# SteveMacenski/slam_toolbox

Measured on AMD Instinct MI355X. Metric: scan-matches/sec, higher is better.
Workload: dtype u8 gather / i32 sum / f64 penalty; 1 GPU; BASELINE config[1]: CorrelateScan 1081 beams 61x61x81 poses; parallelism=1 x independent match shards (no collective), streams_per_gpu=1

## Files before the change

slam_toolbox_amd/csrc/kh_internal.hpp:

```cpp
#pragma once
#include <cstddef>
#include <cstdint>

namespace kh
{

constexpr int32_t kInvalidScan = INT32_MAX;
constexpr int32_t kOccupied = 100;
constexpr int32_t kTieCap = 2048;
constexpr int32_t kGridPad = 512;
constexpr int32_t kTileBytes = 64;
constexpr int32_t kTileSpan = 61;
constexpr int32_t kClasses = 4;
constexpr int32_t kBlockShift = 5;
constexpr int32_t kCountsPerAngle = 8;
#ifndef KH_GROUP_ANGLES
#define KH_GROUP_ANGLES 2
#endif
#ifndef KH_LDS_PITCH
#define KH_LDS_PITCH 192
#endif
#ifndef KH_LDS_ROWS
#define KH_LDS_ROWS 196
#endif
#ifndef KH_LDS_REGION_KB
#define KH_LDS_REGION_KB 37
#endif
constexpr int32_t kGroupAngles = KH_GROUP_ANGLES;
constexpr int32_t kLdsRanges = 4;
inline __host__ __device__ int32_t lds_desc_capacity(int32_t n_points) {return 64 * ((n_points + 255) / 256);}
constexpr int32_t kChunkWords = 8;
static_assert(4 + kGroupAngles <= kChunkWords, "descriptor words");
constexpr int32_t kLdsPitch = KH_LDS_PITCH;
constexpr int32_t kLdsRows = KH_LDS_ROWS;
constexpr int32_t kLdsRegionBytes = KH_LDS_REGION_KB * 1024;

constexpr int32_t kMaxFootprint = 4;
constexpr uint32_t kHashEmpty = 0xffffffffu;
struct RasterJob
{
  uint8_t * grid;
  const double * const * scan_ptr;
  const int32_t * scan_prefix;
  int32_t n_scans;
  int32_t uniform_n;
  double view_x, view_y;
  uint8_t * active;
  int32_t n_points;
  int32_t ws, roi_x, roi_y, roi_w, roi_h;
  int32_t kernel_size;
  double off_x, off_y, scale;
  uint32_t * blockmap;
  int32_t bm_w, bm_h;
  int32_t bshift;
  int32_t tiles_w, tiles_h, height;
  int32_t * tile_count;
  int32_t * tile_start;
  int32_t * tile_cursor;
  int32_t * work;
  int32_t * n_work;
  int32_t * cell_xy;
  int32_t * rank;
  int32_t * list;
  int32_t n_foot;
  int32_t foot_dx[kMaxFootprint], foot_dy[kMaxFootprint];
// ... 110 lines not shown
```

slam_toolbox_amd/csrc/matcher_host.cpp:

```cpp
#include "matcher_private.hpp"
#include "matcher_seq.hpp"

namespace kh
{
thread_local std::string g_last_error;
void set_error(const std::string & s) {g_last_error = s;}
}


namespace kh
{

static int32_t half_kernel_size(double smear, double resolution)
{
  return static_cast<int32_t>(round_half_away(2.0 * smear / resolution));
}


void host_parallel_for(size_t n, const std::function<void(size_t)> & fn) {HostPool::instance().run(n, fn);}
void host_parallel_for_wide(size_t n, const std::function<void(size_t)> & fn) {HostPool::wide().run(n, fn);}
void scan_points_at(const double * ranges, size_t ranges_stride, int32_t n_beams, double min_angle, double angular_resolution, size_t n_poses,
  const double * sensor_poses, double * points, double * sensor_xy)
{
  const size_t nb = static_cast<size_t>(n_beams);
// ... 527 lines not shown
}

int ensure_slot_scratch(kh_matcher * m, const CorrReq & q, CorrHost & c, bool allow_copies)
{
  int rc = KH_OK;
  Slot & s = m->slots[c.slot];
  const size_t tp = static_cast<size_t>(c.na) * c.P;
  if (tp > s.cap_table) {
    if (s.d_table) {KH_HIP(hipStreamSynchronize(m->stream)); KH_HIP(hipFree(s.d_table)); KH_HIP(hipFree(s.d_slow));}
    const size_t cap = std::max(tp, s.cap_table + s.cap_table / 2);
    KH_HIP(hipMalloc(reinterpret_cast<void **>(&s.d_table), cap * 4));
    KH_HIP(hipMalloc(reinterpret_cast<void **>(&s.d_slow), cap * 4));
    s.cap_table = cap;
  }
  rc = ensure_device(s.d_counts, s.cap_counts, static_cast<size_t>(c.na) * kCountsPerAngle, m->stream); if (rc) {return rc;}
  {
    size_t lt = static_cast<size_t>((c.nx + 30) / 31) * ((c.ny + 4 * pick_ry(c.ny) - 1) / (4 * pick_ry(c.ny)));
    if (lt > 32) {lt = 1;}
    c.lt_alloc = static_cast<int32_t>(lt);
    rc = ensure_device(s.d_fast, s.cap_fast, 2 * tp * kClasses * lt, m->stream); if (rc) {return rc;}
    rc = ensure_device(s.d_tcounts, s.cap_tcounts, 2 * static_cast<size_t>(c.na) * kClasses * lt, m->stream); if (rc) {return rc;}
    const double work = static_cast<double>(c.nx) * c.ny * c.na * c.P;
    const double cells_per_step = q.res_x * m->scale;
    const bool full_res = c.nx > 1 && std::fabs(cells_per_step - 1.0) < 1e-9 && c.nx <= kTileSpan;
    const bool tiled_lists = lt > 1 && (std::fabs(cells_per_step - 1.0) < 1e-9 || std::fabs(cells_per_step - 2.0) < 1e-9);
    if (allow_copies && m->dual_copy && !s.d_grid2 && (full_res || tiled_lists) && work >= 1e8) {
      const bool two_cells = std::fabs(cells_per_step - 2.0) < 1e-9 && m->copy_q > 0 && (m->ws % 8) == 0;
      rc = allocate_copies(m, s, two_cells ? 2 : 1); if (rc) {return rc;}
    }
  }
  {
    const size_t groups = (static_cast<size_t>(c.na) + kGroupAngles - 1) / kGroupAngles;
    const size_t range_len = static_cast<size_t>(lds_desc_capacity(c.P));
    rc = ensure_device(s.d_chunks, s.cap_chunks, groups * kLdsRanges * range_len * kChunkWords, m->stream); if (rc) {return rc;}
    rc = ensure_device(s.d_chunk_counts, s.cap_chunk_counts, groups * kLdsRanges, m->stream); if (rc) {return rc;}
  }
  const size_t vol = static_cast<size_t>(c.nx) * c.ny * c.na;
  rc = ensure_device(s.d_sums, s.cap_volume, vol, m->stream); if (rc) {return rc;}
  rc = ensure_device(s.d_tile_best, s.cap_tile_best,
      static_cast<size_t>(c.na) * ((c.nx + 30) / 31) * ((c.ny + 3) / 4), m->stream); if (rc) {return rc;}
  if (m->keep_responses) {rc = ensure_device(s.d_resp, s.cap_resp, vol, m->stream); if (rc) {return rc;}}

  return KH_OK;
}

void prepare_job(kh_matcher * m, const CorrReq & q, CorrHost & c, const StageLayout & L, uint8_t * hb, uint8_t * db,
  unsigned long long * d_out, size_t out_words, size_t n_launch, bool lds_always, bool lds_never, JobShape & shape)
{
  const kh_match_params & mp = m->params;
  Slot & s = m->slots[c.slot];
  CorrJob * job = reinterpret_cast<CorrJob *>(hb);
  int32_t * bx = reinterpret_cast<int32_t *>(hb + L.bx);
  int32_t * by = reinterpret_cast<int32_t *>(hb + L.by);
  double * ang_pen = reinterpret_cast<double *>(hb + L.ang_pen);
  double * cos_sin = reinterpret_cast<double *>(hb + L.cos_sin);
  double * local = reinterpret_cast<double *>(hb + L.local);
  uint8_t * invalid = hb + L.invalid;

  c.bx.resize(c.nx); c.by.resize(c.ny);
  for (int32_t k = 0; k < c.nx; ++k) {
    const double newPositionX = c.center[0] + c.geo->x_poses[k];
    const double gx = (newPositionX - s.off_x) * m->scale;
    c.bx[k] = to_int32(round_half_away(gx)) + m->roi_x;
    bx[k] = c.bx[k];
  }
  for (int32_t k = 0; k < c.ny; ++k) {
    const double newPositionY = c.center[1] + c.geo->y_poses[k];
    const double gy = (newPositionY - s.off_y) * m->scale;
// ... 323 lines not shown
      const CorrJob * job = reinterpret_cast<const CorrJob *>(B.h_stage + stride * i);
      launch_score(B.d_stage + stride * i, stride, 1, job->tiles_x * job->tiles_y, job->na,
        (job->linear && job->sx == 2 && !job->dec) ? 2 : 1, job->ry, cs);
    }
  }
  if (m->profiling) {KH_HIP(hipEventRecord(B.ev[1], cs)); KH_HIP(hipEventRecord(B.evs[2], cs));}
  launch_ties(B.d_stage, stride, static_cast<int32_t>(n), max_poses, tile_pairs, B.use_lds, cs);
  if (m->profiling) {KH_HIP(hipEventRecord(B.evs[3], cs));}
  KH_HIP(hipGetLastError());
  KH_HIP(hipMemcpyAsync(B.h_out, B.d_out, out_words * 8 * n, hipMemcpyDeviceToHost, cs));
  size_t max_small = 0;
  for (size_t i = 0; i < n; ++i) {
    const size_t vol = static_cast<size_t>(B.ctx[i].nx) * B.ctx[i].ny * B.ctx[i].na;
    if (B.ctx[i].fine && vol <= kSmallVolume) {max_small = std::max(max_small, vol);}
  }
  B.small_stride = align_up(max_small, 32);
  if (max_small) {
    rc = ensure_pinned(B.h_sums, B.cap_hsums, B.small_stride * n, m->stream); if (rc) {return rc;}
    rc = ensure_device(B.d_small, B.cap_dsmall, B.small_stride * n, m->stream); if (rc) {return rc;}
    launch_gather_small(B.d_stage, stride, static_cast<int32_t>(n), B.d_small, static_cast<int32_t>(B.small_stride), cs);
    KH_HIP(hipMemcpyAsync(B.h_sums, B.d_small, B.small_stride * n * 4, hipMemcpyDeviceToHost, cs));
  }
  KH_HIP(hipEventRecord(B.done, cs));
  timing.lap(1, t_enqueue);
  return KH_OK;
}

static int dump_lds_chunks(const kh_matcher * m, const CorrBatch & B)
{
  const CorrHost & c0 = B.ctx[0];
  const Slot & s0 = m->slots[c0.slot];
  const size_t groups = (static_cast<size_t>(c0.na) + kGroupAngles - 1) / kGroupAngles;
  const size_t range_len = static_cast<size_t>(lds_desc_capacity(c0.P));
  std::vector<int32_t> cc(groups * kLdsRanges), dd(groups * kLdsRanges * range_len * kChunkWords);
  KH_HIP(hipMemcpy(cc.data(), s0.d_chunk_counts, cc.size() * 4, hipMemcpyDeviceToHost));
  KH_HIP(hipMemcpy(dd.data(), s0.d_chunks, dd.size() * 4, hipMemcpyDeviceToHost));
  long total = 0, bytes = 0, windows = 0, maxb = 0, small = 0;
  for (size_t g = 0; g < groups * kLdsRanges; ++g) {
    for (int32_t k = 0; k < cc[g]; ++k) {
      const int32_t * d = dd.data() + (g * range_len + k) * kChunkWords;
      ++total; bytes += static_cast<long>(d[2]) * kLdsPitch; windows += d[3];
      maxb = std::max<long>(maxb, static_cast<long>(d[2]) * kLdsPitch);
      if (d[3] < 16) {++small;}
    }
  }
  std::fprintf(stderr, "[kh lds] job 0: %zu angle pairs, %ld chunks (%.1f per pair, %ld with < 16 windows), mean region %.1f KB, max %.1f KB, "
    "%.1f windows per chunk, %.0f staged bytes per window\n",
    groups, total, static_cast<double>(total) / groups, small, bytes / 1024.0 / std::max(1l, total), maxb / 1024.0,
    static_cast<double>(windows) / std::max(1l, total), static_cast<double>(bytes) / std::max(1l, windows));
  return KH_OK;
}

static int finish_chunk(kh_matcher * m, CorrReq * reqs, size_t n, CorrBatch & B, bool last_of_call)
{
  if (n == 0) {return KH_OK;}
  StageTiming & timing = stage_timing();
  const auto t_enter = std::chrono::steady_clock::now();
  constexpr uint64_t kAwaitResults = 200 * HostPool::kTicksPerMicrosecond, kAwaitNextCall = 120 * HostPool::kTicksPerMicrosecond;
  if (last_of_call) {HostPool::instance().run(2, [](size_t) {}, kAwaitResults);}
  KH_HIP(hipEventSynchronize(B.done));
  timing.lap(2, t_enter);
  const auto t_final = std::chrono::steady_clock::now();
  if (B.use_lds && std::getenv("KH_LDS_DEBUG")) {
    const int rc = dump_lds_chunks(m, B); if (rc) {return rc;}
  }
  if (m->profiling) {
    float ms = 0;
    KH_HIP(hipEventElapsedTime(&ms, B.ev[0], B.ev[1]));
    m->score_ms += ms; m->score_launches += 1; m->score_jobs += static_cast<int64_t>(n);
    KH_HIP(hipEventElapsedTime(&ms, B.evs[0], B.evs[1])); m->offsets_ms += ms;
    KH_HIP(hipEventElapsedTime(&ms, B.evs[2], B.evs[3])); m->ties_ms += ms;
  }

  std::vector<int> final_rc(n, KH_OK);
  auto finalize = [&](size_t i) -> int {
    const CorrHost & c = B.ctx[i];
    ResultView v;
    v.out = B.h_out + B.out_words * i;
    const size_t vol = static_cast<size_t>(c.nx) * c.ny * c.na;
    v.small = (c.fine && vol <= kSmallVolume && B.h_sums) ? B.h_sums + B.small_stride * i : nullptr;
    v.h_job = reinterpret_cast<CorrJob *>(B.h_stage + B.stride * i); v.d_job = B.d_stage + B.stride * i; v.stride = B.stride;
    return finalize_job(m, reqs[i], B.ctx[i], v);
// ... 707 lines not shown
```

slam_toolbox_amd/csrc/matcher_kernels.hip:

```cpp
#include <hip/hip_runtime.h>
#include <algorithm>
#include <atomic>
#include <cstdint>
#include <cstdlib>
#include "kh_internal.hpp"
#include "matcher_device.hpp"

namespace kh
{

constexpr int kCodeWords = 128;
__global__ __launch_bounds__(64) void k_find_valid_lane(const RasterJob * jobs, const ValidItem * items, int n_items)
{
  __shared__ uint32_t s_codes[kCodeWords][64];
  const int t = blockIdx.x * blockDim.x + threadIdx.x;
  if (t >= n_items) {return;}
  const int lane = threadIdx.x;
  const RasterJob & job = jobs[items[t].job];
  const int k = items[t].scan;
  const int n = job.scan_prefix[k + 1] - job.scan_prefix[k];
  const double2 * pts = reinterpret_cast<const double2 *>(job.scan_ptr[k]);
  uint8_t * out = job.active + job.scan_prefix[k];
  const bool in_lds = n <= 16 * kCodeWords;
  const double vx = job.view_x, vy = job.view_y;
  const double min_square_distance = 0.1 * 0.1;
  double fx = 0.0, fy = 0.0;
  bool first_time = true;
  constexpr int kAhead = 8;
  uint32_t word = 0;
  for (int base = 0; base < n; base += kAhead) {
    double2 c[kAhead];
#pragma unroll
    for (int u = 0; u < kAhead; ++u) {c[u] = pts[min(base + u, n - 1)];}
#pragma unroll
    for (int u = 0; u < kAhead; ++u) {
      const int it = base + u;
      if (it >= n) {break;}
      const double cx = c[u].x, cy = c[u].y;
// ... 1253 lines not shown
          const double delta = response - best;
          const bool tie = delta < 0.0 ? delta >= -1e-06 : delta <= 1e-06;
          if (tie) {
            const unsigned long long slot = atomicAdd(&job.out[1], 1ull);
            if (slot < (unsigned long long)kTieCap) {tie_idx[slot] = (uint32_t)((size_t)p * na + a);}
          }
        }
      }
    }
    __syncthreads();
  }
}

void launch_ties(const uint8_t * d_jobs, size_t stride, int32_t n_jobs, int32_t max_poses, int32_t tile_pairs, bool cells_in_score, void * stream)
{
  if (n_jobs <= 0 || max_poses <= 0) {return;}
  if (cells_in_score) {
    hipLaunchKernelGGL(k_ties_only, dim3(n_jobs >= 16 ? 4 : 16, n_jobs), dim3(256), 0, (hipStream_t)stream, d_jobs, stride);
    return;
  }
  int blocks = (max_poses + 255) / 256;
  if (tile_pairs > 0) {blocks = std::min(tile_pairs, n_jobs >= 16 ? 16 : 64);}
  if (blocks > 1024) {blocks = 1024;}
  hipLaunchKernelGGL(k_ties, dim3(blocks, n_jobs), dim3(256), 0, (hipStream_t)stream, d_jobs, stride);
}

}

namespace kh
{

struct ChunkDesc {int32_t beam_begin, g0, rows, windows, cnt[kChunkWords - 4];};
static_assert(sizeof(ChunkDesc) == kChunkWords * 4, "descriptor size");
static_assert(kGroupAngles >= 2 && kGroupAngles <= 4, "K3' runs kGroupAngles x 4 waves: at most 1024 threads");
static_assert(kLdsPitch % 16 == 0 && kLdsPitch % 128 == 64, "rows of a 32-lane half must fall into disjoint banks");
static_assert(kLdsRegionBytes % 1024 == 0 && kLdsRegionBytes >= kLdsRows * kLdsPitch, "one LDS-DMA instruction fills 1 KB");

constexpr int kNotFast = INT32_MIN;

template <bool kMin>
__device__ __forceinline__ int wave_prefix(int v)
{
  constexpr int ident = kMin ? INT32_MAX : INT32_MIN;
  auto op = [](int x, int y) {return kMin ? (y < x ? y : x) : (y > x ? y : x);};
  v = op(v, __builtin_amdgcn_update_dpp(ident, v, 0x111, 0xf, 0xf, false));
  v = op(v, __builtin_amdgcn_update_dpp(ident, v, 0x112, 0xf, 0xf, false));
  v = op(v, __builtin_amdgcn_update_dpp(ident, v, 0x114, 0xf, 0xf, false));
  v = op(v, __builtin_amdgcn_update_dpp(ident, v, 0x118, 0xf, 0xf, false));
  v = op(v, __builtin_amdgcn_update_dpp(ident, v, 0x142, 0xa, 0xf, false));
  v = op(v, __builtin_amdgcn_update_dpp(ident, v, 0x143, 0xc, 0xf, false));
  return v;
}
__device__ __forceinline__ int wave_prefix_min(int v, int) {return wave_prefix<true>(v);}
__device__ __forceinline__ int wave_prefix_max(int v, int) {return wave_prefix<false>(v);}

__global__ __launch_bounds__(256) void k_offsets_lds(const uint8_t * jobs, size_t stride)
{
  const CorrJob & job = *reinterpret_cast<const CorrJob *>(jobs + (size_t)blockIdx.y * stride);
  const int group = blockIdx.x;
  const int a0 = group * kGroupAngles;
  if (a0 >= job.na) {return;}
  {
    const int groups = (job.na + kGroupAngles - 1) / kGroupAngles;
    const int per = (job.out_words + groups - 1) / groups;
    const int hi = min(job.out_words, (group + 1) * per);
    for (int i = group * per + threadIdx.x; i < hi; i += blockDim.x) {job.out[i] = 0ull;}
  }
  const int P = job.n_points;
  __shared__ int32_t s_slow[kGroupAngles];
  if (threadIdx.x < kGroupAngles) {s_slow[threadIdx.x] = 0;}
  const uint32_t * const bmp = job.blockmap;
  __syncthreads();
  const int lane = threadIdx.x & 63, wave = threadIdx.x >> 6;
  const int64_t bmin = job.base0;
  const int64_t bmax = (int64_t)job.base0 + (int64_t)(job.nx - 1) * job.sx + (int64_t)(job.ny - 1) * job.sy_ws;
  const int32_t xs = (job.nx - 1) * job.sx + 1, ys = (job.ny - 1) * job.sy_cells + 1;
  const int ws = job.ws, bm_w = job.bm_w, bm_h = job.bm_h, bshift = job.bshift, na = job.na, base0 = job.base0;
  const float inv_ws = 1.0f / (float)ws;
  const int64_t data_size = job.data_size, pad = job.pad;
  const double off_x = job.grid_off_x, off_y = job.grid_off_y, scale = job.scale;
  const int row_waves = lds_row_waves(job.ny);
  const int read_rows = (16 * row_waves - 1) * job.sy_cells + 1;
  const int span_rows = ys;
  double cosine[kGroupAngles], sine[kGroupAngles];
#pragma unroll
  for (int q = 0; q < kGroupAngles; ++q) {
    cosine[q] = a0 + q < na ? job.cos_sin[2 * (a0 + q)] : 1.0;
    sine[q] = a0 + q < na ? job.cos_sin[2 * (a0 + q) + 1] : 0.0;
  }
  int32_t * const table = job.table;
  int32_t * const slow = job.slow;
  int32_t * const rel_out = job.rel;
  const int rounds = (P + 255) / 256;
  const int desc_cap = lds_desc_capacity(P);
  ChunkDesc * out = reinterpret_cast<ChunkDesc *>(job.chunks) + ((size_t)group * kLdsRanges + wave) * desc_cap;
  int n_out = 0;
  long long windows_total = 0;
  constexpr int kMaxRounds = 8;
  double plx[kMaxRounds], ply[kMaxRounds];
  bool pinv[kMaxRounds];
  {
    typedef __attribute__((address_space(1))) const uint8_t gflag;
    typedef __attribute__((address_space(1))) const double gdouble;
    gflag * const ginvalid = (gflag *)job.invalid;
    gdouble * const glocal = (gdouble *)job.local;
    uint8_t fl[kMaxRounds];
#pragma unroll
    for (int t = 0; t < kMaxRounds; ++t) {
      const int ic = min((int)threadIdx.x + 256 * t, P - 1);
      fl[t] = ginvalid[ic]; plx[t] = glocal[2 * ic]; ply[t] = glocal[2 * ic + 1];
    }
#pragma unroll
    for (int t = 0; t < kMaxRounds; ++t) {
      const int i = threadIdx.x + 256 * t;
      const bool in = t < rounds && i < P;
      pinv[t] = in ? fl[t] != 0 : true;
      plx[t] = in ? plx[t] : 0.0;
      ply[t] = in ? ply[t] : 0.0;
    }
  }
#pragma unroll
  for (int t = 0; t < kMaxRounds; ++t) {
    if (t >= rounds) {break;}
    const int i = threadIdx.x + 256 * t;
    const bool inr = i < P;
    int gx[kGroupAngles], gy[kGroupAngles];
#pragma unroll
    for (int q = 0; q < kGroupAngles; ++q) {
// ... 57 lines not shown
        const int al = (int)(((int64_t)base0 + xmin) & 15);
        const int px0 = xmin - al;
        const bool fits = any && (xmax - px0 + kTileBytes <= kLdsPitch) && (ymax - ymin + read_rows <= kLdsRows);
        const unsigned long long okm = __ballot(!any || fits) | ((1ull << begin) - 1ull);
        const int first_bad = (okm == ~0ull) ? 64 : __ffsll((long long)~okm) - 1;
        n = first_bad - begin;
        if (n > 0) {
          x0 = __shfl(px0, first_bad - 1); y0 = __shfl(ymin, first_bad - 1);
          rows = __shfl(ymax, first_bad - 1) - y0 + span_rows;
          any_chunk = __shfl((int)any, first_bad - 1) != 0;
          break;
        }
        if (lane == begin) {
          int qd = 0;
#pragma unroll
          for (int q = 1; q < kGroupAngles; ++q) {qd = gy[q] != kNotFast ? q : qd;}
#pragma unroll
          for (int q = 0; q < kGroupAngles; ++q) {
            if (q == qd) {
              (slow + (size_t)(a0 + q) * P)[atomicAdd(&s_slow[q], 1)] = gx[q] + gy[q] * ws;
              gy[q] = kNotFast;
            }
          }
        }
      }
      n = min(n, n_run - begin);
      if (any_chunk) {
        const bool in = lane >= begin && lane < begin + n;
        ChunkDesc d;
        d.beam_begin = run_lo + begin;
        d.g0 = y0 * ws + x0; d.rows = rows;
#pragma unroll
        for (int q = kGroupAngles; q < kChunkWords - 4; ++q) {d.cnt[q] = 0;}
        int windows = 0;
#pragma unroll
        for (int q = 0; q < kGroupAngles; ++q) {
          const int a = a0 + q;
          d.cnt[q] = 0;
          if (a >= na) {continue;}
          const bool mine = in && gy[q] != kNotFast;
          const int rel = (gy[q] - y0) * kLdsPitch + (gx[q] - x0);
          const int cls = rel & 3;
          int offset = 0, my_rank = 0, packed = 0;
#pragma unroll
          for (int c = 0; c < kClasses; ++c) {
            const unsigned long long mask = __ballot(mine && cls == c);
            const int cnt = __popcll(mask);
            if (cls == c) {my_rank = offset + __popcll(mask & ((1ull << lane) - 1ull));}
            offset += cnt;
            packed |= cnt << (8 * c);
          }
          d.cnt[q] = packed;
          windows += offset;
          if (mine) {rel_out[(size_t)a * P + run_lo + begin + my_rank] = rel & ~3;}
        }
        d.windows = windows;
        windows_total += windows;
        if (lane == 0) {out[n_out] = d;}
        ++n_out;
      }
      begin += n;
    }
  }
  if (lane == 0) {
    job.chunk_counts[(size_t)group * kLdsRanges + wave] = n_out;
    if (job.load_counter && windows_total) {atomicAdd(job.load_counter, (unsigned long long)(windows_total * 4 * row_waves));}
  }
  __syncthreads();
  if (threadIdx.x < kGroupAngles && a0 + (int)threadIdx.x < job.na) {
    job.counts[kCountsPerAngle * (a0 + threadIdx.x) + kClasses] = s_slow[threadIdx.x];
  }
}

void launch_offsets_lds(const uint8_t * d_jobs, size_t stride, int32_t n_jobs, int32_t max_na, void * stream)
{
  if (n_jobs <= 0 || max_na <= 0) {return;}
  const int groups = (max_na + kGroupAngles - 1) / kGroupAngles;
  hipLaunchKernelGGL(k_offsets_lds, dim3(groups, n_jobs), dim3(256), 0, (hipStream_t)stream, d_jobs, stride);
}

typedef __attribute__((address_space(3))) uint32_t lds_u32;
typedef __attribute__((address_space(1))) const void gvoid;
typedef int v4i __attribute__((ext_vector_type(4)));

#ifndef KH_PRIO
#define KH_PRIO 1
#endif
constexpr int kScoreLdsBlocksPerCu = (160 * 1024 - 4096) / (2 * kLdsRegionBytes);
constexpr int kTilePoses = 64 * kTileSpan;
static_assert(kGroupAngles * kTilePoses * 4 + (kGroupAngles - 1) * kTilePoses * 8 <= 2 * kLdsRegionBytes,
  "the sums and the exchanged responses of kGroupAngles angles must fit the workgroup's two LDS regions");
static_assert((kGroupAngles * kTilePoses * 4) % 8 == 0, "the exchanged responses are doubles");
static_assert(kScoreLdsBlocksPerCu >= 1 && kScoreLdsBlocksPerCu * kGroupAngles * 4 <= 16, "four waves per SIMD");
template <int S, int NW, bool kFull>
__global__ __launch_bounds__(64 * kGroupAngles * NW, 4) void k_score_lds(const uint8_t * jobs, size_t stride, int n_jobs, int groups_max, int xcd_map)
{
  constexpr int RQ = 16 / NW;
  constexpr int kThreadsPerAngle = 64 * NW;
  constexpr int PX = (S == 1) ? kTileSpan : (kTileSpan + 1) / 2;
  constexpr int kRowStep = 4 * S * kLdsPitch;
  int job_index, group;
  if (xcd_map) {
    const int xcd = blockIdx.x & 7, qb = blockIdx.x >> 3;
    job_index = (qb / groups_max) * 8 + xcd;
// ... 7 lines not shown
  if (group * kGroupAngles >= job.na) {return;}
  extern __shared__ __attribute__((aligned(16))) uint32_t s_region[];
  const int tid = threadIdx.x;
  const int lane = tid & 63;
  const int wave = __builtin_amdgcn_readfirstlane(tid >> 6);
  const int lx = lane & 15, ly = lane >> 4;
  const int q = wave / NW, quarter = wave % NW;
  const int row_waves = kFull ? NW : lds_row_waves(job.ny) * (NW / 4);
  const int parts = kFull ? 1 : NW / row_waves;
  const int share = kFull ? quarter : quarter % row_waves, part = kFull ? 0 : quarter / row_waves;
  const int a = group * kGroupAngles + q;
  const bool live = a < job.na;
  const int P = job.n_points;
  const int range_len = lds_desc_capacity(P);

  v4i acc[kClasses][RQ];
#pragma unroll
  for (int c = 0; c < kClasses; ++c) {
#pragma unroll
    for (int r = 0; r < RQ; ++r) {acc[c][r] = v4i{0, 0, 0, 0};}
  }
  v4i sel;
  {
    const int i = lane & 15;
    const int one = ((lane >> 4) == (i >> 2)) ? (int)(0x01010101u & (0xffu << (8 * (i & 3)))) : 0;
    sel = v4i{one, one, one, one};
  }
  const int lanebase = 4 * lx + (4 * RQ * share + ly) * S * kLdsPitch;

  const gbyte * gwin = as_global(job.grid) + job.base0;
  const gint * grel = as_global(job.rel + (size_t)(live ? a : 0) * P);
  typedef const __attribute__((address_space(4))) int32_t cint;
  cint * cdescs = (cint *)(job.chunks + (size_t)group * kLdsRanges * range_len * kChunkWords);
  cint * ccounts = (cint *)(job.chunk_counts + (size_t)group * kLdsRanges);
  struct Chunk {int beam_begin, g0, rows, packed;};

  constexpr int kUnitsPerRow = kLdsPitch / 16;
  constexpr int kWaves = kGroupAngles * NW;
  constexpr int kDmaPerWave = (kLdsRegionBytes / 1024 + kWaves - 1) / kWaves;
  const int ws = job.ws;
  uint32_t dma_off[kDmaPerWave];
#pragma unroll
  for (int t = 0; t < kDmaPerWave; ++t) {
    const int u = 64 * (wave + kWaves * t) + lane;
    const int row = u / kUnitsPerRow, col = u - row * kUnitsPerRow;
    dma_off[t] = (uint32_t)(row * ws + 16 * col);
  }
  auto issue_dma = [&](const Chunk & d, int buf) {
    const gbyte * src = gwin + d.g0;
    const int nblk = (d.rows * kUnitsPerRow + 63) >> 6;
    const uint32_t o_last = (uint32_t)((d.rows - 1) * ws + 16 * (kUnitsPerRow - 1));
    lds_u32 * dst = (lds_u32 *)s_region + buf * (kLdsRegionBytes / 4) + wave * 256;
#pragma unroll
    for (int t = 0; t < kDmaPerWave; ++t) {
      if (wave + kWaves * t >= nblk) {break;}
      const uint32_t o = dma_off[t] < o_last ? dma_off[t] : o_last;
      __builtin_amdgcn_global_load_lds((gvoid *)(src + o), (__attribute__((address_space(3))) void *)(dst + kWaves * t * 256), 16, 0, 0);
    }
  };
  auto load_rel = [&](const Chunk & d) -> int32_t {
    const int cnt = (d.packed & 0xff) + ((d.packed >> 8) & 0xff) + ((d.packed >> 16) & 0xff) + ((d.packed >> 24) & 0xff);
    return (live && lane < cnt) ? grel[d.beam_begin + lane] : 0;
  };
  const uint32_t lds_base = (uint32_t)(uintptr_t)(__attribute__((address_space(3))) char *)((char *)s_region);
  const uint32_t lds_lane = lds_base + (uint32_t)lanebase;
#define KH_DSR(dst, addr, r) asm volatile("ds_read_b32 %0, %1 offset:%2" : "=v"(dst) : "v"(addr), "n"((r) * kRowStep) : "memory")
#define KH_STEP(selector) do { \
    int32_t w[RQ][4]; \
    _Pragma("unroll") for (int r = 0; r < RQ; ++r) {KH_DSR(w[r][0], a0, r); KH_DSR(w[r][1], a1, r); KH_DSR(w[r][2], a2, r); KH_DSR(w[r][3], a3, r);} \
    if (RQ == 4) { \
      asm volatile("s_waitcnt lgkmcnt(0)" : "+v"(w[0][0]), "+v"(w[0][1]), "+v"(w[0][2]), "+v"(w[0][3]), "+v"(w[1][0]), "+v"(w[1][1]), "+v"(w[1][2]), "+v"(w[1][3]), \
        "+v"(w[RQ - 2][0]), "+v"(w[RQ - 2][1]), "+v"(w[RQ - 2][2]), "+v"(w[RQ - 2][3]), "+v"(w[RQ - 1][0]), "+v"(w[RQ - 1][1]), "+v"(w[RQ - 1][2]), "+v"(w[RQ - 1][3])); \
    } else { \
      asm volatile("s_waitcnt lgkmcnt(0)" : "+v"(w[0][0]), "+v"(w[0][1]), "+v"(w[0][2]), "+v"(w[0][3]), "+v"(w[1][0]), "+v"(w[1][1]), "+v"(w[1][2]), "+v"(w[1][3])); \
    } \
    _Pragma("unroll") for (int r = 0; r < RQ; ++r) { \
      acc[c][r] = __builtin_amdgcn_mfma_i32_16x16x64_i8(selector, (v4i{w[r][0], w[r][1], w[r][2], w[r][3]}), acc[c][r], 0, 0, 0); \
    } \
  } while (0)
  int step_base = 0;
  auto score = [&](const Chunk & d, int buf, int32_t rels) {
    if (!live) {return;}
    const uint32_t base = lds_lane + (uint32_t)(buf * kLdsRegionBytes);
    int off = 0;
#pragma unroll
    for (int c = 0; c < kClasses; ++c) {
      const int cnt = (d.packed >> (8 * c)) & 0xff;
      const int first = kFull ? 0 : (part - step_base) & (parts - 1);
      if (!kFull) {step_base += (cnt + 3) >> 2;}
      int k = 4 * first;
      for (; k + 4 <= cnt; k += 4 * parts) {
        const int i0 = off + k;
        const uint32_t a0 = base + (uint32_t)__builtin_amdgcn_readlane(rels, i0);
        const uint32_t a1 = base + (uint32_t)__builtin_amdgcn_readlane(rels, i0 + 1);
        const uint32_t a2 = base + (uint32_t)__builtin_amdgcn_readlane(rels, i0 + 2);
        const uint32_t a3 = base + (uint32_t)__builtin_amdgcn_readlane(rels, i0 + 3);
        KH_STEP(sel);
      }
      if (k < cnt) {
        const int i0 = off + k, rem = cnt - k;
        const uint32_t a0 = base + (uint32_t)__builtin_amdgcn_readlane(rels, i0);
        const uint32_t a1 = base + (uint32_t)__builtin_amdgcn_readlane(rels, rem > 1 ? i0 + 1 : i0);
        const uint32_t a2 = base + (uint32_t)__builtin_amdgcn_readlane(rels, rem > 2 ? i0 + 2 : i0);
        const uint32_t a3 = a0;
        const v4i sel_tail = v4i{sel[0], rem > 1 ? sel[1] : 0, rem > 2 ? sel[2] : 0, 0};
        KH_STEP(sel_tail);
      }
      off += cnt;
    }
  };
#undef KH_STEP
#undef KH_DSR

  static_assert(kLdsRanges == 4, "the four chunk counts are held in scalar registers");
  const int end0 = ccounts[0], end1 = end0 + ccounts[1], end2 = end1 + ccounts[2], n_chunks = end2 + ccounts[3];
  int fetched = 0;
  auto next_chunk = [&](Chunk & d) -> bool {
    if (fetched >= n_chunks) {return false;}
    const int range = (fetched >= end0 ? 1 : 0) + (fetched >= end1 ? 1 : 0) + (fetched >= end2 ? 1 : 0);
    const int start = fetched >= end2 ? end2 : fetched >= end1 ? end1 : fetched >= end0 ? end0 : 0;
    cint * w = cdescs + ((size_t)range * range_len + (fetched - start)) * kChunkWords;
    d.beam_begin = w[0]; d.g0 = w[1]; d.rows = w[2]; d.packed = w[4 + q];
    ++fetched;
    return true;
  };
  Chunk cur = {0, 0, 0, 0}, nxt = {0, 0, 0, 0}, aft = {0, 0, 0, 0};
  bool have = next_chunk(cur);
  bool more = have && next_chunk(nxt);
  int buf = 0;
  int32_t rel_cur = 0, rel_nxt = 0;
  if (have) {issue_dma(cur, 0); rel_cur = load_rel(cur);}
  while (have) {
    __syncthreads();
    if (more) {issue_dma(nxt, buf ^ 1); rel_nxt = load_rel(nxt);}
    const bool after = more && next_chunk(aft);
    __builtin_amdgcn_s_setprio(KH_PRIO);
    score(cur, buf, rel_cur);
    __builtin_amdgcn_s_setprio(0);
    cur = nxt; nxt = aft; rel_cur = rel_nxt; buf ^= 1; have = more; more = after;
  }
  __syncthreads();

  const size_t plane = (size_t)job.nx * job.ny;
  const int ta = tid % kThreadsPerAngle;
  int32_t * s_tile = reinterpret_cast<int32_t *>(s_region) + q * (64 * PX);
  if (S == 1 && kFull) {
    if (live) {
#pragma unroll
      for (int r = 0; r < RQ; ++r) {
        int32_t * const row = s_tile + (4 * RQ * share + 4 * r + ly) * PX + 4 * lx;
#pragma unroll
        for (int b = 0; b < 4; ++b) {
          int32_t total = acc[0][r][b];
#pragma unroll
          for (int c = 1; c < kClasses; ++c) {
            const int32_t v = acc[c][r][(b + c) & 3];
            total += (b + c) < 4 ? v : __builtin_amdgcn_update_dpp(0, v, 0x101, 0xf, 0xf, true);
          }
          if (4 * lx + b < PX) {row[b] = total;}
        }
      }
    }
  } else {
    for (int i = ta; i < 64 * PX; i += kThreadsPerAngle) {s_tile[i] = 0;}
    __syncthreads();
    if (live) {
#pragma unroll
      for (int c = 0; c < kClasses; ++c) {
#pragma unroll
        for (int r = 0; r < RQ; ++r) {
#pragma unroll
          for (int b = 0; b < 4; ++b) {
            const int j = 4 * lx + b;
            const int x = (j - c) / S;
            const bool pose = j >= c && ((j - c) % S) == 0 && x < PX;
            if (pose && acc[c][r][b] != 0) {atomicAdd(&s_tile[(4 * RQ * share + 4 * r + ly) * PX + x], acc[c][r][b]);}
          }
        }
      }
    }
  }
  constexpr int kPosesPerThread = (64 * PX + kThreadsPerAngle - 1) / kThreadsPerAngle;
  const int nx = job.nx, ny = job.ny;
  const bool penal = job.do_penalize != 0, wr_resp = job.write_resp != 0;
  const double denom = job.denom;
  int32_t * const sums_out = job.sums + (size_t)(live ? a : 0) * plane;
  double * const resp_out = wr_resp ? job.resp + (size_t)(live ? a : 0) * plane : nullptr;
  const int32_t * const jbx = job.bx, * const jby = job.by;
  const uint8_t * const jgrid = job.grid;
  const int64_t data_size = job.data_size;
  constexpr int kOwned = (kPosesPerThread + kGroupAngles - 1) / kGroupAngles;
  constexpr int kRounds = kOwned * kGroupAngles;
  const bool cells = job.coarse != 0 && job.cells_in_score != 0;
  typedef __attribute__((address_space(1))) unsigned long long gu64;
  gu64 * const probs = (gu64 *)(job.out + kOutHeaderWords);
  double * const s_xch = reinterpret_cast<double *>(reinterpret_cast<int32_t *>(s_region) + kGroupAngles * kTilePoses);
  auto slab_of = [&](int owner) -> int {return kGroupAngles == 2 ? 0 : (q - owner + kGroupAngles) % kGroupAngles - 1;};
  double dpen[kRounds];
  const double apen = (live && penal) ? job.ang_pen[a] : 1.0;
#pragma unroll
  for (int k = 0; k < kRounds; ++k) {
    const int p = ta + kThreadsPerAngle * k;
    const int yi = p / PX, xi = p % PX;
    dpen[k] = (live && penal && xi < nx && yi < ny) ? job.dist_pen[yi * nx + xi] : 1.0;
  }
  double mine[kOwned];
#pragma unroll
  for (int j = 0; j < kOwned; ++j) {mine[j] = 0.0;}
  __syncthreads();
  const int n_slow = live ? job.counts[kCountsPerAngle * a + kClasses] : 0;
  const int32_t * slow = job.slow + (size_t)(live ? a : 0) * P;
  double best = 0.0;
#pragma unroll
  for (int k = 0; k < kRounds; ++k) {
    const int p = ta + kThreadsPerAngle * k;
    const int yi = p / PX, xi = p % PX;
    if (xi >= nx || yi >= ny) {continue;}
    const bool owned = k % kGroupAngles == q;
    double response = 0.0;
    if (live) {
      int32_t sum = s_tile[p];
      if (n_slow > 0) {
        const int64_t pose = (int64_t)jbx[xi] + (int64_t)jby[yi];
        for (int j = 0; j < n_slow; ++j) {
          const int64_t idx = pose + slow[j];
          if (idx >= 0 && idx < data_size) {sum += jgrid[idx];}
        }
      }
      const size_t o = (size_t)yi * nx + xi;
      sums_out[o] = sum;
      response = (double)sum / denom;
      if (penal) {
        const double delta = response - 0.0;
        const bool is_zero = delta < 0.0 ? delta >= -1e-06 : delta <= 1e-06;
        if (!is_zero) {response *= (dpen[k] * apen);}
      }
      if (wr_resp) {resp_out[o] = response;}
      best = response > best ? response : best;
    }
    if (cells) {
      if (owned) {mine[k / kGroupAngles] = response;} else {s_xch[slab_of(k % kGroupAngles) * kTilePoses + p] = response;}
    }
  }
  unsigned long long seen[kOwned];
  uint32_t cell[kOwned];
  constexpr uint32_t kNoCell = 0xffffffffu;
#pragma unroll
  for (int j = 0; j < kOwned; ++j) {
    const int p = ta + kThreadsPerAngle * (kGroupAngles * j + q);
    const int yi = p / PX, xi = p % PX;
    cell[j] = (cells && xi < nx && yi < ny) ? (uint32_t)(yi * nx + xi) : kNoCell;
    __builtin_assume(cell[j] == kNoCell || cell[j] < 64u * kTileSpan);
    seen[j] = cell[j] != kNoCell ? __hip_atomic_load(probs + cell[j], __ATOMIC_RELAXED, __HIP_MEMORY_SCOPE_AGENT) : 0ull;
  }
#pragma unroll
  for (int sft = 32; sft > 0; sft >>= 1) {
    const double o = __shfl_xor(best, sft);
    best = o > best ? o : best;
  }
  __shared__ double s_best[kGroupAngles * NW];
  if (lane == 0) {s_best[wave] = best;}
  __syncthreads();
  if (live && ta == 0) {
    const double * wb = s_best + NW * q;
    double b = wb[0];
#pragma unroll
    for (int t = 1; t < NW; ++t) {b = wb[t] > b ? wb[t] : b;}
    if (job.tile_best) {job.tile_best[a] = b;}
    if (b > 0.0) {atomicMax(&job.out[0], (unsigned long long)__double_as_longlong(b));}
  }
  if (cells) {
    bool raise[kOwned];
#pragma unroll
    for (int j = 0; j < kOwned; ++j) {
      const int p = ta + kThreadsPerAngle * (kGroupAngles * j + q);
      raise[j] = false;
      if (cell[j] == kNoCell) {continue;}
#pragma unroll
      for (int t = 0; t < kGroupAngles - 1; ++t) {
        const double o = s_xch[t * kTilePoses + p];
        mine[j] = o > mine[j] ? o : mine[j];
      }
      raise[j] = (unsigned long long)__double_as_longlong(mine[j]) > seen[j];
    }
#pragma unroll
    for (int j = 0; j < kOwned; ++j) {
      if (raise[j]) {
        (void)__hip_atomic_fetch_max(probs + cell[j], (unsigned long long)__double_as_longlong(mine[j]), __ATOMIC_RELAXED, __HIP_MEMORY_SCOPE_AGENT);
      }
    }
  }
}

void launch_score_lds(const uint8_t * d_jobs, size_t stride, int32_t n_jobs, int32_t max_na, int32_t sx_variant, bool full_rows, void * stream)
{
  if (n_jobs <= 0 || max_na <= 0) {return;}
  const int groups = (max_na + kGroupAngles - 1) / kGroupAngles;
  const int xcd_map = n_jobs >= 8 ? 1 : 0;
  const int jobs_per_xcd = (n_jobs + 7) / 8;
  const long long blocks = xcd_map ? 8ll * jobs_per_xcd * groups : (long long)n_jobs * groups;
  constexpr int kDyn = 2 * kLdsRegionBytes;
  static std::atomic<unsigned long long> attr_done[4] = {{0}, {0}, {0}, {0}};
// ... 16 lines not shown
```

Baseline: 120,400 scan-matches/s.

## Stage LDS chunks through a variable-size ring with deeper DMA prefetch

Replaces the fixed double-buffered LDS staging in the scoring kernel with a ring allocator that places each chunk by its actual size. This lets up to two chunks be prefetched ahead using counted vmcnt waits instead of full syncthreads. The offsets kernel now compacts the per-wave descriptor lists into one flat list per group, and precomputes DMA unit counts and last offsets so each descriptor arrives in one scalar load. Relative-offset loads also move to LDS via DMA, and the cell atomic loads are hoisted earlier. This adds a compaction pass, doubles the descriptor buffer, and relies on hand-tuned wait counts and ring-overlap logic, which could race if the accounting is wrong.

```diff
diff --git a/slam_toolbox_amd/csrc/kh_internal.hpp b/slam_toolbox_amd/csrc/kh_internal.hpp
--- a/slam_toolbox_amd/csrc/kh_internal.hpp
+++ b/slam_toolbox_amd/csrc/kh_internal.hpp
@@ -29,8 +29,8 @@
 constexpr int32_t kGroupAngles = KH_GROUP_ANGLES;
 constexpr int32_t kLdsRanges = 4;
 inline __host__ __device__ int32_t lds_desc_capacity(int32_t n_points) {return 64 * ((n_points + 255) / 256);}
-constexpr int32_t kChunkWords = 8;
-static_assert(4 + kGroupAngles <= kChunkWords, "descriptor words");
+constexpr int32_t kChunkWords = kGroupAngles <= 2 ? 8 : 16;
+static_assert(4 + kGroupAngles + 2 <= kChunkWords, "descriptor words");
 constexpr int32_t kLdsPitch = KH_LDS_PITCH;
 constexpr int32_t kLdsRows = KH_LDS_ROWS;
 constexpr int32_t kLdsRegionBytes = KH_LDS_REGION_KB * 1024;
diff --git a/slam_toolbox_amd/csrc/lds_ring.hpp b/slam_toolbox_amd/csrc/lds_ring.hpp
--- /dev/null
+++ b/slam_toolbox_amd/csrc/lds_ring.hpp
@@ -0,0 +1,27 @@
+#pragma once
+#include <cstdint>
+
+#if defined(__HIPCC__)
+#define KH_RING_FN __host__ __device__ inline
+#else
+#define KH_RING_FN inline
+#endif
+
+namespace kh
+{
+
+struct RingPlace {int32_t unit; bool fits;};
+
+KH_RING_FN RingPlace lds_ring_place(int32_t ring_half, int32_t off_old, int32_t n_old, int32_t off_new, int32_t n_new, int32_t n)
+{
+  int32_t at = n_new > 0 ? off_new + n_new : 0;
+  if (at < ring_half && at + n > ring_half) {at = ring_half;}
+  if (at + n > 2 * ring_half) {at = 0;}
+  const bool hits_old = n_old > 0 && at < off_old + n_old && off_old < at + n;
+  const bool hits_new = n_new > 0 && at < off_new + n_new && off_new < at + n;
+  return RingPlace{at, !hits_old && !hits_new};
+}
+
+KH_RING_FN int32_t lds_ring_units(int32_t rows, int32_t pitch) {return (rows * pitch + 1023) >> 10;}
+
+}
diff --git a/slam_toolbox_amd/csrc/matcher_host.cpp b/slam_toolbox_amd/csrc/matcher_host.cpp
--- a/slam_toolbox_amd/csrc/matcher_host.cpp
+++ b/slam_toolbox_amd/csrc/matcher_host.cpp
@@ -583,8 +583,8 @@
   {
     const size_t groups = (static_cast<size_t>(c.na) + kGroupAngles - 1) / kGroupAngles;
     const size_t range_len = static_cast<size_t>(lds_desc_capacity(c.P));
-    rc = ensure_device(s.d_chunks, s.cap_chunks, groups * kLdsRanges * range_len * kChunkWords, m->stream); if (rc) {return rc;}
-    rc = ensure_device(s.d_chunk_counts, s.cap_chunk_counts, groups * kLdsRanges, m->stream); if (rc) {return rc;}
+    rc = ensure_device(s.d_chunks, s.cap_chunks, 2 * groups * kLdsRanges * range_len * kChunkWords, m->stream); if (rc) {return rc;}
+    rc = ensure_device(s.d_chunk_counts, s.cap_chunk_counts, groups, m->stream); if (rc) {return rc;}
   }
   const size_t vol = static_cast<size_t>(c.nx) * c.ny * c.na;
   rc = ensure_device(s.d_sums, s.cap_volume, vol, m->stream); if (rc) {return rc;}
@@ -974,13 +974,14 @@
   const Slot & s0 = m->slots[c0.slot];
   const size_t groups = (static_cast<size_t>(c0.na) + kGroupAngles - 1) / kGroupAngles;
   const size_t range_len = static_cast<size_t>(lds_desc_capacity(c0.P));
-  std::vector<int32_t> cc(groups * kLdsRanges), dd(groups * kLdsRanges * range_len * kChunkWords);
+  const size_t group_len = kLdsRanges * range_len;
+  std::vector<int32_t> cc(groups), dd(groups * group_len * kChunkWords);
   KH_HIP(hipMemcpy(cc.data(), s0.d_chunk_counts, cc.size() * 4, hipMemcpyDeviceToHost));
   KH_HIP(hipMemcpy(dd.data(), s0.d_chunks, dd.size() * 4, hipMemcpyDeviceToHost));
   long total = 0, bytes = 0, windows = 0, maxb = 0, small = 0;
-  for (size_t g = 0; g < groups * kLdsRanges; ++g) {
+  for (size_t g = 0; g < groups; ++g) {
     for (int32_t k = 0; k < cc[g]; ++k) {
-      const int32_t * d = dd.data() + (g * range_len + k) * kChunkWords;
+      const int32_t * d = dd.data() + (g * group_len + k) * kChunkWords;
       ++total; bytes += static_cast<long>(d[2]) * kLdsPitch; windows += d[3];
       maxb = std::max<long>(maxb, static_cast<long>(d[2]) * kLdsPitch);
       if (d[3] < 16) {++small;}
@@ -990,6 +991,14 @@
     "%.1f windows per chunk, %.0f staged bytes per window\n",
     groups, total, static_cast<double>(total) / groups, small, bytes / 1024.0 / std::max(1l, total), maxb / 1024.0,
     static_cast<double>(windows) / std::max(1l, total), static_cast<double>(bytes) / std::max(1l, windows));
+  for (size_t g = 0; g < groups; ++g) {
+    std::fprintf(stderr, "[kh lds] job 0 pair %zu:", g);
+    for (int32_t k = 0; k < cc[g]; ++k) {
+      const int32_t * d = dd.data() + (g * group_len + k) * kChunkWords;
+      std::fprintf(stderr, " %d:%d:%d:%d:%d", d[0], d[2], d[3], d[kChunkWords - 2], d[kChunkWords - 1]);
+    }
+    std::fprintf(stderr, "\n");
+  }
   return KH_OK;
 }
 
diff --git a/slam_toolbox_amd/csrc/matcher_kernels.hip b/slam_toolbox_amd/csrc/matcher_kernels.hip
--- a/slam_toolbox_amd/csrc/matcher_kernels.hip
+++ b/slam_toolbox_amd/csrc/matcher_kernels.hip
@@ -4,6 +4,7 @@
 #include <cstdint>
 #include <cstdlib>
 #include "kh_internal.hpp"
+#include "lds_ring.hpp"
 #include "matcher_device.hpp"
 
 namespace kh
@@ -1323,6 +1324,7 @@
 
 struct ChunkDesc {int32_t beam_begin, g0, rows, windows, cnt[kChunkWords - 4];};
 static_assert(sizeof(ChunkDesc) == kChunkWords * 4, "descriptor size");
+constexpr int kDescUnits = kChunkWords - 2, kDescLast = kChunkWords - 1;
 static_assert(kGroupAngles >= 2 && kGroupAngles <= 4, "K3' runs kGroupAngles x 4 waves: at most 1024 threads");
 static_assert(kLdsPitch % 16 == 0 && kLdsPitch % 128 == 64, "rows of a 32-lane half must fall into disjoint banks");
 static_assert(kLdsRegionBytes % 1024 == 0 && kLdsRegionBytes >= kLdsRows * kLdsPitch, "one LDS-DMA instruction fills 1 KB");
@@ -1359,6 +1361,7 @@
   }
   const int P = job.n_points;
   __shared__ int32_t s_slow[kGroupAngles];
+  __shared__ int32_t s_nout[kLdsRanges];
   if (threadIdx.x < kGroupAngles) {s_slow[threadIdx.x] = 0;}
   const uint32_t * const bmp = job.blockmap;
   __syncthreads();
@@ -1384,7 +1387,9 @@
   int32_t * const rel_out = job.rel;
   const int rounds = (P + 255) / 256;
   const int desc_cap = lds_desc_capacity(P);
-  ChunkDesc * out = reinterpret_cast<ChunkDesc *>(job.chunks) + ((size_t)group * kLdsRanges + wave) * desc_cap;
+  const int groups_all = (na + kGroupAngles - 1) / kGroupAngles;
+  ChunkDesc * const flat = reinterpret_cast<ChunkDesc *>(job.chunks) + (size_t)group * kLdsRanges * desc_cap;
+  ChunkDesc * out = reinterpret_cast<ChunkDesc *>(job.chunks) + ((size_t)(groups_all + group) * kLdsRanges + wave) * desc_cap;
   int n_out = 0;
   long long windows_total = 0;
   constexpr int kMaxRounds = 8;
@@ -1508,6 +1513,8 @@
         d.g0 = y0 * ws + x0; d.rows = rows;
 #pragma unroll
         for (int q = kGroupAngles; q < kChunkWords - 4; ++q) {d.cnt[q] = 0;}
+        d.cnt[kDescUnits - 4] = lds_ring_units(rows, kLdsPitch);
+        d.cnt[kDescLast - 4] = (rows - 1) * ws + 16 * (kLdsPitch / 16 - 1);
         int windows = 0;
 #pragma unroll
         for (int q = 0; q < kGroupAngles; ++q) {
@@ -1539,13 +1546,28 @@
     }
   }
   if (lane == 0) {
-    job.chunk_counts[(size_t)group * kLdsRanges + wave] = n_out;
+    s_nout[wave] = n_out;
     if (job.load_counter && windows_total) {atomicAdd(job.load_counter, (unsigned long long)(windows_total * 4 * row_waves));}
   }
   __syncthreads();
   if (threadIdx.x < kGroupAngles && a0 + (int)threadIdx.x < job.na) {
     job.counts[kCountsPerAngle * (a0 + threadIdx.x) + kClasses] = s_slow[threadIdx.x];
   }
+  int before = 0, total = 0;
+#pragma unroll
+  for (int w = 0; w < kLdsRanges; ++w) {
+    const int n = s_nout[w];
+    before += w < wave ? n : 0; total += n;
+  }
+  {
+    typedef int v4i32 __attribute__((ext_vector_type(4)));
+    static_assert(sizeof(ChunkDesc) % 16 == 0, "descriptors are moved 16 bytes at a time");
+    constexpr int kPer = sizeof(ChunkDesc) / 16;
+    const v4i32 * const src = reinterpret_cast<const v4i32 *>(out);
+    v4i32 * const dst = reinterpret_cast<v4i32 *>(flat + before);
+    for (int k = lane; k < kPer * n_out; k += 64) {dst[k] = src[k];}
+  }
+  if (threadIdx.x == 0) {job.chunk_counts[group] = total;}
 }
 
 void launch_offsets_lds(const uint8_t * d_jobs, size_t stride, int32_t n_jobs, int32_t max_na, void * stream)
@@ -1619,8 +1641,9 @@
   const gint * grel = as_global(job.rel + (size_t)(live ? a : 0) * P);
   typedef const __attribute__((address_space(4))) int32_t cint;
   cint * cdescs = (cint *)(job.chunks + (size_t)group * kLdsRanges * range_len * kChunkWords);
-  cint * ccounts = (cint *)(job.chunk_counts + (size_t)group * kLdsRanges);
-  struct Chunk {int beam_begin, g0, rows, packed;};
+  const int n_chunks = ((cint *)job.chunk_counts)[group];
+  const int n_slow = live ? ((cint *)job.counts)[kCountsPerAngle * a + kClasses] : 0;
+  struct Chunk {int beam_begin, g0, cnt[kGroupAngles], units, o_last, at;};
 
   constexpr int kUnitsPerRow = kLdsPitch / 16;
   constexpr int kWaves = kGroupAngles * NW;
@@ -1633,22 +1656,24 @@
     const int row = u / kUnitsPerRow, col = u - row * kUnitsPerRow;
     dma_off[t] = (uint32_t)(row * ws + 16 * col);
   }
-  auto issue_dma = [&](const Chunk & d, int buf) {
+  __shared__ int32_t s_rel[3][kGroupAngles][64];
+  const int rel_last = P - 1;
+  auto issue_dma = [&](const Chunk & d, int slot) {
+    if (live && quarter == 0) {
+      const int i = min(d.beam_begin + lane, rel_last);
+      __builtin_amdgcn_global_load_lds((gvoid *)(grel + i), (__attribute__((address_space(3))) void *)&s_rel[slot][q][0], 4, 0, 0);
+    }
     const gbyte * src = gwin + d.g0;
-    const int nblk = (d.rows * kUnitsPerRow + 63) >> 6;
-    const uint32_t o_last = (uint32_t)((d.rows - 1) * ws + 16 * (kUnitsPerRow - 1));
-    lds_u32 * dst = (lds_u32 *)s_region + buf * (kLdsRegionBytes / 4) + wave * 256;
+    const uint32_t o_last = (uint32_t)d.o_last;
+    lds_u32 * dst = (lds_u32 *)s_region + d.at * 256 + wave * 256;
 #pragma unroll
     for (int t = 0; t < kDmaPerWave; ++t) {
-      if (wave + kWaves * t >= nblk) {break;}
+      if (wave + kWaves * t >= d.units) {break;}
       const uint32_t o = dma_off[t] < o_last ? dma_off[t] : o_last;
       __builtin_amdgcn_global_load_lds((gvoid *)(src + o), (__attribute__((address_space(3))) void *)(dst + kWaves * t * 256), 16, 0, 0);
     }
   };
-  auto load_rel = [&](const Chunk & d) -> int32_t {
-    const int cnt = (d.packed & 0xff) + ((d.packed >> 8) & 0xff) + ((d.packed >> 16) & 0xff) + ((d.packed >> 24) & 0xff);
-    return (live && lane < cnt) ? grel[d.beam_begin + lane] : 0;
-  };
+  auto dma_pieces = [&](const Chunk & d) -> int {return max(0, (d.units - wave + kWaves - 1) / kWaves);};
   const uint32_t lds_base = (uint32_t)(uintptr_t)(__attribute__((address_space(3))) char *)((char *)s_region);
   const uint32_t lds_lane = lds_base + (uint32_t)lanebase;
 #define KH_DSR(dst, addr, r) asm volatile("ds_read_b32 %0, %1 offset:%2" : "=v"(dst) : "v"(addr), "n"((r) * kRowStep) : "memory")
@@ -1666,13 +1691,16 @@
     } \
   } while (0)
   int step_base = 0;
-  auto score = [&](const Chunk & d, int buf, int32_t rels) {
+  auto score = [&](const Chunk & d, int32_t rels) {
     if (!live) {return;}
-    const uint32_t base = lds_lane + (uint32_t)(buf * kLdsRegionBytes);
+    int packed = d.cnt[0];
+#pragma unroll
+    for (int t = 1; t < kGroupAngles; ++t) {packed = q == t ? d.cnt[t] : packed;}
+    const uint32_t base = lds_lane + (uint32_t)(d.at * 1024);
     int off = 0;
 #pragma unroll
     for (int c = 0; c < kClasses; ++c) {
-      const int cnt = (d.packed >> (8 * c)) & 0xff;
+      const int cnt = (packed >> (8 * c)) & 0xff;
       const int first = kFull ? 0 : (part - step_base) & (parts - 1);
       if (!kFull) {step_base += (cnt + 3) >> 2;}
       int k = 4 * first;
@@ -1699,37 +1727,82 @@
 #undef KH_STEP
 #undef KH_DSR
 
-  static_assert(kLdsRanges == 4, "the four chunk counts are held in scalar registers");
-  const int end0 = ccounts[0], end1 = end0 + ccounts[1], end2 = end1 + ccounts[2], n_chunks = end2 + ccounts[3];
+  constexpr int kRingHalf = kLdsRegionBytes / 1024;
+  static_assert(kDmaPerWave <= 5, "the counted waits below");
+  typedef int v8i __attribute__((ext_vector_type(8)));
+  static_assert(kChunkWords == 8, "a descriptor is one scalar load of eight words");
   int fetched = 0;
   auto next_chunk = [&](Chunk & d) -> bool {
     if (fetched >= n_chunks) {return false;}
-    const int range = (fetched >= end0 ? 1 : 0) + (fetched >= end1 ? 1 : 0) + (fetched >= end2 ? 1 : 0);
-    const int start = fetched >= end2 ? end2 : fetched >= end1 ? end1 : fetched >= end0 ? end0 : 0;
-    cint * w = cdescs + ((size_t)range * range_len + (fetched - start)) * kChunkWords;
-    d.beam_begin = w[0]; d.g0 = w[1]; d.rows = w[2]; d.packed = w[4 + q];
+    const v8i w = *(const __attribute__((address_space(4))) v8i *)(cdescs + (size_t)fetched * kChunkWords);
+    d.beam_begin = w[0]; d.g0 = w[1];
+#pragma unroll
+    for (int t = 0; t < kGroupAngles; ++t) {d.cnt[t] = w[4 + t];}
+    d.units = w[kDescUnits]; d.o_last = w[kDescLast]; d.at = 0;
     ++fetched;
     return true;
   };
-  Chunk cur = {0, 0, 0, 0}, nxt = {0, 0, 0, 0}, aft = {0, 0, 0, 0};
-  bool have = next_chunk(cur);
-  bool more = have && next_chunk(nxt);
-  int buf = 0;
-  int32_t rel_cur = 0, rel_nxt = 0;
-  if (have) {issue_dma(cur, 0); rel_cur = load_rel(cur);}
-  while (have) {
-    __syncthreads();
-    if (more) {issue_dma(nxt, buf ^ 1); rel_nxt = load_rel(nxt);}
-    const bool after = more && next_chunk(aft);
+  const uint32_t rel_lane = (uint32_t)(uintptr_t)(__attribute__((address_space(3))) char *)((char *)&s_rel[0][q][lane]);
+  Chunk c0 = {}, c1 = c0, c2 = c0, c3 = c0;
+  bool h0 = next_chunk(c0);
+  bool h1 = h0 && next_chunk(c1);
+  bool h2 = h1 && next_chunk(c2);
+  bool issued1 = false;
+  int slot = 0;
+  int ahead = 0;
+  if (h0) {issue_dma(c0, 0);}
+  while (h0) {
+    switch (ahead) {
+      case 0: asm volatile("s_waitcnt vmcnt(0)" ::: "memory"); break;
+      case 1: asm volatile("s_waitcnt vmcnt(1)" ::: "memory"); break;
+      case 2: asm volatile("s_waitcnt vmcnt(2)" ::: "memory"); break;
+      case 3: asm volatile("s_waitcnt vmcnt(3)" ::: "memory"); break;
+      case 4: asm volatile("s_waitcnt vmcnt(4)" ::: "memory"); break;
+      default: asm volatile("s_waitcnt vmcnt(5)" ::: "memory"); break;
+    }
+    __builtin_amdgcn_s_barrier();
+    int32_t rels;
+    asm volatile("ds_read_b32 %0, %1" : "=v"(rels) : "v"(rel_lane + (uint32_t)(slot * (int)sizeof(s_rel[0]))) : "memory");
+    const bool h3 = h2 && next_chunk(c3);
+    const int slot1 = slot == 2 ? 0 : slot + 1, slot2 = slot1 == 2 ? 0 : slot1 + 1;
+    if (h1 && !issued1) {
+      c1.at = lds_ring_place(kRingHalf, 0, 0, c0.at, c0.units, c1.units).unit;
+      issue_dma(c1, slot1);
+    }
+    ahead = 0;
+    bool issued2 = false;
+    if (h2) {
+      const RingPlace place = lds_ring_place(kRingHalf, c0.at, c0.units, c1.at, c1.units, c2.units);
+      if (place.fits) {c2.at = place.unit; issue_dma(c2, slot2); ahead = dma_pieces(c2); issued2 = true;}
+    }
+    asm volatile("s_waitcnt lgkmcnt(0)" : "+v"(rels) :: "memory");
     __builtin_amdgcn_s_setprio(KH_PRIO);
-    score(cur, buf, rel_cur);
+    score(c0, rels);
     __builtin_amdgcn_s_setprio(0);
-    cur = nxt; nxt = aft; rel_cur = rel_nxt; buf ^= 1; have = more; more = after;
+    c0 = c1; c1 = c2; c2 = c3; h0 = h1; h1 = h2; h2 = h3; issued1 = issued2; slot = slot1;
   }
   __syncthreads();
 
-  const size_t plane = (size_t)job.nx * job.ny;
+  const __attribute__((address_space(4))) CorrJob & cj = *(const __attribute__((address_space(4))) CorrJob *)(jobs + (size_t)job_index * stride);
+  const int nx = cj.nx, ny = cj.ny;
+  const size_t plane = (size_t)nx * ny;
   const int ta = tid % kThreadsPerAngle;
+  constexpr int kPosesPerThread = (64 * PX + kThreadsPerAngle - 1) / kThreadsPerAngle;
+  constexpr int kOwned = (kPosesPerThread + kGroupAngles - 1) / kGroupAngles;
+  const bool cells = cj.coarse != 0 && cj.cells_in_score != 0;
+  typedef __attribute__((address_space(1))) unsigned long long gu64;
+  gu64 * const probs = (gu64 *)(cj.out + kOutHeaderWords);
+  unsigned long long seen[kOwned];
+  uint32_t cell[kOwned];
+  constexpr uint32_t kNoCell = 0xffffffffu;
+#pragma unroll
+  for (int j = 0; j < kOwned; ++j) {
+    const int p = ta + kThreadsPerAngle * (kGroupAngles * j + q);
+    const int yi = p / PX, xi = p % PX;
+    cell[j] = (cells && xi < nx && yi < ny) ? (uint32_t)(yi * nx + xi) : kNoCell;
+    __builtin_assume(cell[j] == kNoCell || cell[j] < 64u * kTileSpan);
+    seen[j] = cell[j] != kNoCell ? __hip_atomic_load(probs + cell[j], __ATOMIC_RELAXED, __HIP_MEMORY_SCOPE_AGENT) : 0ull;
+  }
   int32_t * s_tile = reinterpret_cast<int32_t *>(s_region) + q * (64 * PX);
   if (S == 1 && kFull) {
     if (live) {
@@ -1767,36 +1840,38 @@
       }
     }
   }
-  constexpr int kPosesPerThread = (64 * PX + kThreadsPerAngle - 1) / kThreadsPerAngle;
-  const int nx = job.nx, ny = job.ny;
-  const bool penal = job.do_penalize != 0, wr_resp = job.write_resp != 0;
-  const double denom = job.denom;
-  int32_t * const sums_out = job.sums + (size_t)(live ? a : 0) * plane;
-  double * const resp_out = wr_resp ? job.resp + (size_t)(live ? a : 0) * plane : nullptr;
-  const int32_t * const jbx = job.bx, * const jby = job.by;
-  const uint8_t * const jgrid = job.grid;
-  const int64_t data_size = job.data_size;
-  constexpr int kOwned = (kPosesPerThread + kGroupAngles - 1) / kGroupAngles;
+  const bool penal = cj.do_penalize != 0, wr_resp = cj.write_resp != 0;
+  const double denom = cj.denom;
+  int32_t * const sums_out = cj.sums + (size_t)(live ? a : 0) * plane;
+  double * const resp_out = wr_resp ? cj.resp + (size_t)(live ? a : 0) * plane : nullptr;
+  const int32_t * const jbx = cj.bx, * const jby = cj.by;
+  const uint8_t * const jgrid = cj.grid;
+  const int64_t data_size = cj.data_size;
   constexpr int kRounds = kOwned * kGroupAngles;
-  const bool cells = job.coarse != 0 && job.cells_in_score != 0;
-  typedef __attribute__((address_space(1))) unsigned long long gu64;
-  gu64 * const probs = (gu64 *)(job.out + kOutHeaderWords);
   double * const s_xch = reinterpret_cast<double *>(reinterpret_cast<int32_t *>(s_region) + kGroupAngles * kTilePoses);
   auto slab_of = [&](int owner) -> int {return kGroupAngles == 2 ? 0 : (q - owner + kGroupAngles) % kGroupAngles - 1;};
   double dpen[kRounds];
-  const double apen = (live && penal) ? job.ang_pen[a] : 1.0;
-#pragma unroll
-  for (int k = 0; k < kRounds; ++k) {
-    const int p = ta + kThreadsPerAngle * k;
-    const int yi = p / PX, xi = p % PX;
-    dpen[k] = (live && penal && xi < nx && yi < ny) ? job.dist_pen[yi * nx + xi] : 1.0;
+  typedef __attribute__((address_space(1))) const double gdouble;
+  double apen = 1.0;
+#pragma unroll
+  for (int k = 0; k < kRounds; ++k) {dpen[k] = 1.0;}
+  if (live && penal) {
+    gdouble * const gdist = (gdouble *)cj.dist_pen;
+    apen = ((gdouble *)cj.ang_pen)[a];
+#pragma unroll
+    for (int k = 0; k < kRounds; ++k) {
+      const int p = ta + kThreadsPerAngle * k;
+      const int yi = p / PX, xi = p % PX;
+      const bool in = xi < nx && yi < ny;
+      const double v = gdist[in ? yi * nx + xi : 0];
+      dpen[k] = in ? v : 1.0;
+    }
   }
   double mine[kOwned];
 #pragma unroll
   for (int j = 0; j < kOwned; ++j) {mine[j] = 0.0;}
   __syncthreads();
-  const int n_slow = live ? job.counts[kCountsPerAngle * a + kClasses] : 0;
-  const int32_t * slow = job.slow + (size_t)(live ? a : 0) * P;
+  const int32_t * slow = cj.slow + (size_t)(live ? a : 0) * P;
   double best = 0.0;
 #pragma unroll
   for (int k = 0; k < kRounds; ++k) {
@@ -1829,17 +1904,6 @@
       if (owned) {mine[k / kGroupAngles] = response;} else {s_xch[slab_of(k % kGroupAngles) * kTilePoses + p] = response;}
     }
   }
-  unsigned long long seen[kOwned];
-  uint32_t cell[kOwned];
-  constexpr uint32_t kNoCell = 0xffffffffu;
-#pragma unroll
-  for (int j = 0; j < kOwned; ++j) {
-    const int p = ta + kThreadsPerAngle * (kGroupAngles * j + q);
-    const int yi = p / PX, xi = p % PX;
-    cell[j] = (cells && xi < nx && yi < ny) ? (uint32_t)(yi * nx + xi) : kNoCell;
-    __builtin_assume(cell[j] == kNoCell || cell[j] < 64u * kTileSpan);
-    seen[j] = cell[j] != kNoCell ? __hip_atomic_load(probs + cell[j], __ATOMIC_RELAXED, __HIP_MEMORY_SCOPE_AGENT) : 0ull;
-  }
 #pragma unroll
   for (int sft = 32; sft > 0; sft >>= 1) {
     const double o = __shfl_xor(best, sft);
@@ -1853,8 +1917,8 @@
     double b = wb[0];
 #pragma unroll
     for (int t = 1; t < NW; ++t) {b = wb[t] > b ? wb[t] : b;}
-    if (job.tile_best) {job.tile_best[a] = b;}
-    if (b > 0.0) {atomicMax(&job.out[0], (unsigned long long)__double_as_longlong(b));}
+    if (cj.tile_best) {cj.tile_best[a] = b;}
+    if (b > 0.0) {atomicMax(&cj.out[0], (unsigned long long)__double_as_longlong(b));}
   }
   if (cells) {
     bool raise[kOwned];
```

Result: slower. 114,600 scan-matches/s (-4.8%).
